# Nick-qsv/MLP-PPO-2PLY-P3

Measured on AMD Instinct MI355X. Metric: self-play env steps/sec (whole node) + 2-ply evals/sec at batch=65536, higher is better.
Workload: dtype int8 boards / fp32-equivalent policy MLP (split-f16 MFMA); 1 GPU; C3: B=65536 games/GPU PPO rollout step (policy 198->128->{500,1} + masked sample + env.step, rollout rows stored to an HBM ring); global_batch=65536, games_per_gpu=65536, max_legal_moves=500, parallelism=dp1 (independent game shards), streams_per_gpu=4, step_fork=False

## Files before the change

### mlp-ppo-2ply-p3_amd/csrc/bg_debug.h

```cpp
#pragma once
#include <string>

std::string bgx_dbg(const char* name);
long long bgx_dbg_int(const char* name, long long dflt);
```

### mlp-ppo-2ply-p3_amd/csrc/bg_engine.hip

```cpp
#include <hip/hip_runtime.h>
#include <stdio.h>
#include <stdint.h>
#include <string.h>
#include <stdlib.h>
#include <algorithm>
#include <cmath>
#include <mutex>
#include <string>
#include <vector>

#include "bg_engine.h"
#include "bg_rollout.h"
#include "bg_debug.h"
#include "bg_host.h"
#include <map>

using namespace bg;

namespace {

constexpr int kMaxRegions = BGX_MAX_COPY_REGIONS;
using namespace bg;

template <int PHASE, int LOG, int MEMO, bool NO_DOUBLES = false, int DICE = -1, bool BLK = false>
// ... 558 lines not shown
    }
    for_each_group(fin, g, [&](int gl, bool mine, uint64_t m) {
        int64_t* row = tally + (size_t)gl * 8;
        tally_add(row, BGX_ROLLOUT_GAMES, (long long)__popcll(m));
        tally_add(row, BGX_ROLLOUT_PLIES, wave_sum(mine ? p : 0));
        #pragma unroll
        for (int f = BGX_ROLLOUT_WIN1; f <= BGX_ROLLOUT_LOSS3; ++f) tally_add(row, f, count(mine && field == f));
    });
    tally_add(active, 0, -count(retired));
}

__global__ __launch_bounds__(256) void k_rollout_luck_add(const uint8_t* recs, const uint8_t* starts,
                                                          const int32_t* plies, const uint8_t* sel, const float* luck,
                                                          int n, float* lane_luck) {
    const int i = blockIdx.x * 256 + threadIdx.x;
    if (i >= n || !sel[i]) return;
    if (plies[i] == 0 && starts[(size_t)i * 64 + R_ROLL0] != 0) return;
    const float l = luck[i];
    lane_luck[i] += recs[(size_t)i * 64 + R_CUR] == starts[(size_t)i * 64 + R_CUR] ? l : -l;
}

__global__ __launch_bounds__(256) void k_rollout_luck_flush(const uint8_t* starts, const int32_t* group,
                                                            const uint8_t* sel, const uint8_t* done,
                                                            const int32_t* info, int n, int n_groups,
                                                            float* lane_luck, int64_t* luck_tally) {
    const int i = blockIdx.x * 256 + threadIdx.x;
    const bool on = i < n && sel[i] != 0;
    const int g = on ? rollout_group(group, i, n_groups) : -1;
    const bool dn = on && done[i] != 0;
    int winner, score;
    result_of(dn ? info[i] : 0, &winner, &score);
    const bool fin = dn && g >= 0 && winner >= 0;
    long long lq = 0, res = 0;
    if (fin) {
        lq = luck_q(lane_luck[i]);
        res = winner == (int)(starts[(size_t)i * 64 + R_CUR] & 1) ? score : -score;
    }
    if (dn) lane_luck[i] = 0.0f;
    for_each_group(fin, g, [&](int gl, bool mine, uint64_t m) {
        const long long v = mine ? lq : 0;
        int64_t* row = luck_tally + (size_t)gl * 4;
        tally_add(row, BGX_ROLLOUT_LUCK, wave_sum(v));
        tally_add(row, BGX_ROLLOUT_LUCK2, wave_sum(v * v));
        tally_add(row, BGX_ROLLOUT_RESLUCK, wave_sum(mine ? res * lq : 0));
        tally_add(row, BGX_ROLLOUT_LUCK_GAMES, (long long)__popcll(m));
    });
}

__device__ __forceinline__ uint64_t mix64(uint64_t x) {
    x ^= x >> 33; x *= 0xFF51AFD7ED558CCDull;
    x ^= x >> 33; x *= 0xC4CEB9FE1A85EC53ull;
    x ^= x >> 33;
    return x;
}

__global__ __launch_bounds__(256) void k_random_act(const uint8_t* recs, int n, uint64_t seed, uint32_t step,
                                                    int32_t* act) {
    const int i = blockIdx.x * 256 + threadIdx.x;
    if (i >= n) return;
    const uint32_t cnt = (uint32_t)recs[(size_t)i * 64 + R_NM0] | ((uint32_t)recs[(size_t)i * 64 + R_NM1] << 8);
    const uint64_t h = mix64(mix64(seed ^ 0x9E3779B97F4A7C15ull) + (((uint64_t)step << 32) | (uint32_t)i));
    act[i] = (int32_t)(((h >> 32) * (uint64_t)cnt) >> 32);
}

thread_local std::string g_err;

}

int bgx_internal_fail(hipError_t e, int code) {
    g_err = hipGetErrorString(e);
    return code;
}
void bgx_set_error(const char* msg) { g_err = msg; }
static std::mutex g_dbg_mu;
static std::map<std::string, std::string> g_dbg;
std::string bgx_dbg(const char* name) {
    std::lock_guard<std::mutex> g(g_dbg_mu);
    const auto it = g_dbg.find(name);
    return it == g_dbg.end() ? std::string() : it->second;
}
long long bgx_dbg_int(const char* name, long long dflt) {
    const std::string v = bgx_dbg(name);
    return v.empty() ? dflt : strtoll(v.c_str(), nullptr, 10);
}

#define LAUNCH_LOG(K, grid, s, ...) hipLaunchKernelGGL(K<9>, grid, dim3(64), 0, s, __VA_ARGS__)

static void launch_count(bgx_engine* e, hipStream_t s) {
    const int ncnt = (e->a.B + kCountThreads - 1) / kCountThreads;
    hipLaunchKernelGGL(k_order_count, dim3(ncnt), dim3(kCountThreads), 0, s, e->a.pre, e->a.cls, e->a.ctr, e->a.key0, e->a.key1,
                       e->order_cnt, e->a.B, e->ovf_base + 4 * (e->ovf_parity ^ 1), e->a.xcd);
    e->ovf_next_zeroed = true;
    e->gather_due = true;
}

static void launch_gather(bgx_engine* e, hipStream_t s, const int32_t* actions) {
    const Args& A = e->a;
    const int nblk = (A.B + kGatherThreads - 1) / kGatherThreads, ncnt = (A.B + kCountThreads - 1) / kCountThreads;
    if (actions)
        hipLaunchKernelGGL(k_step_gather<true>, dim3(nblk), dim3(kGatherThreads), 0, s, A.cls, e->order_cnt, e->perm, A.B,
                           ncnt, A.xcd, A.moves, A.ctr, actions, A.max_moves, e->blk);
    else
        hipLaunchKernelGGL(k_step_gather<false>, dim3(nblk), dim3(kGatherThreads), 0, s, A.cls, e->order_cnt, e->perm, A.B,
                           ncnt, A.xcd, nullptr, nullptr, nullptr, 0, nullptr);
}

struct StepIo {
    const int32_t* actions;
    float *obs, *reward;
    uint8_t* done;
    int32_t* info;
};

static void launch_heavy(hipStream_t s, const Args& a, int grid, const StepIo& io) {
    if (grid <= 0) return;
    if (a.blk)
        hipLaunchKernelGGL((k_step<0, 9, 0, false, 1, BGX_DICE_PHILOX, true>), dim3(grid), dim3(64), 0, s, a, io.actions,
                           io.obs, io.reward, io.done, io.info, 0);
    else if (a.dice_mode == BGX_DICE_PHILOX)
        hipLaunchKernelGGL((k_step<0, 9, 0, false, 1, BGX_DICE_PHILOX>), dim3(grid), dim3(64), 0, s, a, io.actions,
                           io.obs, io.reward, io.done, io.info, 0);
    else
        hipLaunchKernelGGL((k_step<0, 9, 0>), dim3(grid), dim3(64), 0, s, a, io.actions, io.obs, io.reward, io.done,
                           io.info, 0);
}

static void launch_light(hipStream_t s, const Args& a, int heavy, const StepIo& io) {
    hipLaunchKernelGGL((k_step<0, 8, 0, true, 1, BGX_DICE_PHILOX, true>), dim3(a.B - heavy), dim3(64), 0, s, a, io.actions,
                       io.obs, io.reward, io.done, io.info, heavy);
}

static int heavy_grid(int B, bool xcd) {
    const double g = B / 6.0 + 4.0 * std::sqrt(B * 5.0 / 36.0) + 32.0;
    int h = g >= B ? B : (int)g;
    if (xcd) h = (h + 7) & ~7;
    return h > B ? B : h;
}

static int slow_path(bgx_engine* e, hipStream_t s, int src, const int8_t* boards, const uint8_t* players,
                     const uint8_t* dice, int cap, int16_t* nm, int32_t* nt, uint64_t* moves) {
    if (src == 0)
        hipLaunchKernelGGL(k_movegen_over<0>, dim3(e->slow_waves), dim3(64), 0, s, e->a, boards, players, dice, cap,
                           nm, nt, moves, e->slow_tables);
    else
        hipLaunchKernelGGL(k_movegen_over<1>, dim3(e->slow_waves), dim3(64), 0, s, e->a, boards, players, dice, cap,
                           nm, nt, moves, e->slow_tables);
    return bgx_launch_status();
}

struct EngineBuf {
    void** p;
    size_t bytes;
    bool zero;
};
static std::vector<EngineBuf> engine_bufs(bgx_engine* e, bool stamps, bool order) {
    Args& A = e->a;
    const size_t B = (size_t)A.B;
    const bool shared = A.dice_mode == BGX_DICE_MT_SHARED;
    return {
        {(void**)&A.lanes, B * 64, true},
        {(void**)&A.moves, B * (size_t)A.max_moves * 8, false},
        {(void**)&A.n_total, B * 4, true},
        {(void**)&A.mt, (A.dice_mode == BGX_DICE_MT_LANE ? B : 1) * kMtWords * 4, false},
        {(void**)&A.ctr, B * 8, true},
        {(void**)&A.shared_rolls, B * 4, false},
        {(void**)&e->ovf_base, 32, true},
// ... 578 lines not shown
```

### mlp-ppo-2ply-p3_amd/csrc/bg_mlp.hip

```cpp
#include <hip/hip_runtime.h>
#include <stdint.h>
#include <stdlib.h>
#include "bg_host.h"
#include "bg_debug.h"


namespace {

constexpr int kW1Ahead = 2;

typedef float f32x16 __attribute__((ext_vector_type(16)));
typedef _Float16 f16x8 __attribute__((ext_vector_type(8)));

constexpr int kIn = 198;
constexpr int kKB1 = (kIn + 15) / 16;
constexpr float kMaskLog = -103.27892990343185f;
constexpr int kHdr = 16;

__device__ __forceinline__ int lane_id() { return threadIdx.x & 63; }

__host__ __device__ inline int kperm_src(int kb, int h, int i) {
    if (kb < 12) {
        const int p = kb >= 6 ? 1 : 0;
        const int pt = 4 * (kb - 6 * p) + 2 * h + (i >> 2);
// ... 12 lines not shown
            const int n = rec[base + q];
            f[4 * q + 0] = n >= 1 ? (_Float16)1.0f : (_Float16)0.0f;
            f[4 * q + 1] = n >= 2 ? (_Float16)1.0f : (_Float16)0.0f;
            f[4 * q + 2] = n >= 3 ? (_Float16)1.0f : (_Float16)0.0f;
            f[4 * q + 3] = (_Float16)(n >= 3 ? (float)(n - 3) * 0.5f : 0.0f);
        }
    } else {
        const bool on = h == 0;
        f[0] = on ? (_Float16)((float)rec[48] * 0.5f) : (_Float16)0.0f;
        f[1] = on ? (_Float16)(float)rec[50] : (_Float16)0.0f;
        f[2] = on ? (_Float16)((float)rec[49] * 0.5f) : (_Float16)0.0f;
        f[3] = on ? (_Float16)(float)rec[51] : (_Float16)0.0f;
        f[4] = on && rec[52] == 0 ? (_Float16)1.0f : (_Float16)0.0f;
        f[5] = on && rec[52] != 0 ? (_Float16)1.0f : (_Float16)0.0f;
        f[6] = (_Float16)0.0f;
        f[7] = (_Float16)0.0f;
    }
    return f;
}

__device__ __forceinline__ void split(float x, _Float16& hi, _Float16& lo) {
    hi = (_Float16)x;
    lo = (_Float16)(x - (float)hi);
}

__device__ __forceinline__ f16x8 as_h8(uint4 v) { return __builtin_bit_cast(f16x8, v); }

__device__ __forceinline__ int scale_exp(float max_abs) {
    if (!(max_abs > 0.0f) || !(max_abs < INFINITY)) return 0;
    int q;
    (void)frexpf(max_abs, &q);
    const int e = 14 - q;
    return e < -100 ? -100 : (e > 100 ? 100 : e);
}

__device__ __forceinline__ uint32_t mix32(uint32_t x) {
    x ^= x >> 16; x *= 0x7FEB352Du; x ^= x >> 15; x *= 0x846CA68Bu; x ^= x >> 16;
    return x;
}

__device__ __forceinline__ float fast_ln(float x) { return __builtin_amdgcn_logf(x) * 0.69314718055994531f; }
__device__ __forceinline__ float fast_exp(float x) { return __builtin_amdgcn_exp2f(x * 1.4426950408889634f); }

constexpr float kGumbelMax = 17.0f;

__device__ __forceinline__ float gumbel(uint32_t w) {
    const float u = ((float)(w >> 9) + 0.5f) * (1.0f / 8388608.0f);
    const float v = 1.0f - u;
    const float series = v * (1.0f + v * (0.5f + v * (1.0f / 3.0f)));
    const float e = v < (1.0f / 64.0f) ? series : -fast_ln(u);
    return -fast_ln(e);
}

__device__ __forceinline__ int hid(int r, int h) { return (r & 3) + 8 * (r >> 2) + 4 * h; }

struct PackView {
    const int* hdr;
    const uint4* w1q;
    const float* b1p;
    const uint4* w2q;
    const float* b2p;
};

__host__ __device__ inline int sz_w1q(int T) { return kKB1 * T * 2 * 64 * 4; }
__host__ __device__ inline int sz_b1p(int T) { return T * 16 * 64; }
__host__ __device__ inline int sz_w2q(int T, int OT) { return OT * T * 2 * 2 * 64 * 4; }
__host__ __device__ inline int sz_b2p(int OT) { return OT * 16 * 64; }

template <typename P>
__host__ __device__ inline void views(P base, int T, int OT, P& hdr, P& w1q, P& b1p, P& w2q, P& b2p) {
    hdr = base;
    w1q = hdr + kHdr;
    b1p = w1q + sz_w1q(T);
    w2q = b1p + sz_b1p(T);
    b2p = w2q + sz_w2q(T, OT);
}

constexpr int kZWin = 256, kZCap = 64;
constexpr int kHeavyDefault = 64;
constexpr int kRowBestDefault = 2;

#ifdef BGX_POLICY_STAMPS
constexpr int kStampWaves = 8192;
__device__ unsigned long long g_pstamp[kStampWaves][6];
#define PSTAMP(k) do { if (MODE == 0 && sw < kStampWaves && lane_id() == 0) g_pstamp[sw][k] = __builtin_amdgcn_s_memrealtime(); } while (0)
#else
#define PSTAMP(k) do { } while (0)
#endif
constexpr float kSkipMargin = 30.0f;

template <int T, int MODE>
__global__ __launch_bounds__(MODE == 0 ? 256 : 64) __attribute__((amdgpu_waves_per_eu(2))) void k_policy_act(const uint8_t* __restrict__ recs, int n,
                                                   const float* __restrict__ packed, int n_actions, int n_otiles,
                                                   uint32_t seed_lo, uint32_t seed_hi, uint32_t step_arg,
                                                   const uint32_t* __restrict__ step_ctr, int greedy_arg,
                                                   int32_t* act_out, float* logp_out, float* value_out,
                                                   float* logits_arg, uint8_t* records_out, int skip_arg) {
#ifdef BGX_POLICY_STAMPS
    const int sw = (int)(blockIdx.x * (MODE == 0 ? 4 : 1) + (threadIdx.x >> 6));
#endif
    PSTAMP(0);
    const uint32_t step = step_arg + (step_ctr ? *step_ctr : 0u);
    constexpr int kW = MODE == 0 ? 4 : 1;
    const bool greedy = MODE < 0 ? (greedy_arg & 1) != 0 : false;
    const int rowbest = (greedy_arg >> 1) & 3;
    float* const logits_out = MODE < 0 ? logits_arg : nullptr;
    const bool skip_on = MODE == 0 && skip_arg != 0;
    __shared__ uint8_t srec_[kW][32 * 64];
    __shared__ int zl[MODE == 0 ? kZCap : 1];
    const float *hdrf, *w1f, *b1p, *w2f, *b2p;
    views(packed, T, n_otiles, hdrf, w1f, b1p, w2f, b2p);
    const uint4* w1q = (const uint4*)w1f;
    const uint4* w2q = (const uint4*)w2f;
    const int e1 = __builtin_bit_cast(int, hdrf[0]), e2 = __builtin_bit_cast(int, hdrf[1]);
    const int l = lane_id();
    const int j = l & 31, h = l >> 5;
    const int wv = kW > 1 ? __builtin_amdgcn_readfirstlane((int)(threadIdx.x >> 6)) : 0;
    uint8_t* const srec = srec_[wv];
    const int n_extra = skip_on ? 2 * ((n + kZWin - 1) / kZWin) : 0;
    const bool extra = (int)blockIdx.x < n_extra;
    const int row0 = (((int)blockIdx.x - n_extra) * kW + wv) * 32;
    if (!extra && row0 >= n) return;
    int nzw = 0;
    if (skip_on) {
        const int base = (extra ? (int)blockIdx.x >> 1 : row0 / kZWin) * kZWin;
        uint16_t cw[kZWin / 64];
        #pragma unroll
        for (int k = 0; k < kZWin / 64; ++k)
            cw[k] = *(const uint16_t*)(recs + (size_t)min(base + 64 * k + l, n - 1) * 64 + 60);
        #pragma unroll
        for (int k = 0; k < kZWin / 64; ++k) {
            const int r = base + 64 * k + l;
            const bool z = r < n && (cw[k] == 0 || (int)cw[k] > skip_arg);
            const uint64_t m = __ballot(z);
            const int pos = nzw + __popcll(m & ((1ull << l) - 1ull));
            if (extra && wv == 0 && z && pos < kZCap) zl[pos] = r;
            nzw += __popcll(m);
        }
    }
    const int kx = extra ? ((int)blockIdx.x & 1) : 0;
    const int nz = extra ? min(nzw - 32 * kx, 32) : 32;
    if (extra && (nzw > kZCap || nz <= 0)) return;
    const bool self_zero = skip_on && !extra && nzw > kZCap;
    const int vt = n_actions >> 5;
    if (extra) __syncthreads();
    {
        const int r = l >> 1, off = (l & 1) * 32;
        const int gr = extra ? zl[32 * kx + (r < nz ? r : 0)] : (row0 + r < n ? row0 + r : n - 1);
        const uint4* src = (const uint4*)(recs + (size_t)gr * 64 + off);
        uint4* dst = (uint4*)(srec + r * 64 + off);
        const uint4 v0 = src[0], v1 = src[1];
        dst[0] = v0;
        dst[1] = v1;
        if (!extra && records_out && row0 + r < n) {
            uint4* o = (uint4*)(records_out + (size_t)(row0 + r) * 64 + off);
            o[0] = v0;
            o[1] = v1;
        }
    }
    if (kW > 1) __builtin_amdgcn_wave_barrier(); else __syncthreads();
    const uint8_t* myrec = srec + j * 64;
    const int count = (int)myrec[60] | ((int)myrec[61] << 8);
    const bool gathered = skip_on && !extra && !self_zero && (count == 0 || count > skip_arg);
    const bool row_ok = extra ? j < nz : row0 + j < n;
    const int grow = extra ? zl[32 * kx + (j < nz ? j : 0)] : row0 + j;
    const int per = extra ? (n_otiles + kW - 1) / kW : n_otiles;
    const int o_beg = extra ? min(wv * per, n_otiles) : 0, o_end = extra ? min(o_beg + per, n_otiles) : n_otiles;

    PSTAMP(1);
    f32x16 x1[T];
    constexpr int kPD = kW1Ahead;
    if (kW > 1 && extra) {
        f32x16 acc;
        if (wv < T) {
            #pragma unroll
            for (int r = 0; r < 16; ++r) acc[r] = b1p[(wv * 16 + r) * 64 + l];
            uint4 wr[kPD + 1][2];
            #pragma unroll
            for (int p = 0; p < kPD; ++p)
                #pragma unroll
                for (int f = 0; f < 2; ++f) wr[p][f] = w1q[(p * 2 * T + 2 * wv + f) * 64 + l];
            #pragma unroll
            for (int kb = 0; kb < kKB1; ++kb) {
                if (kb + kPD < kKB1) {
                    #pragma unroll
                    for (int f = 0; f < 2; ++f)
                        wr[(kb + kPD) % (kPD + 1)][f] = w1q[((kb + kPD) * 2 * T + 2 * wv + f) * 64 + l];
                }
                __builtin_amdgcn_sched_barrier(0);
                const f16x8 bf = feats8(myrec, kb, h);
                acc = __builtin_amdgcn_mfma_f32_32x32x16_f16(as_h8(wr[kb % (kPD + 1)][1]), bf, acc, 0, 0, 0);
                acc = __builtin_amdgcn_mfma_f32_32x32x16_f16(as_h8(wr[kb % (kPD + 1)][0]), bf, acc, 0, 0, 0);
            }
        }
        float* const xs = (float*)&srec_[0][0];
        #pragma unroll
        for (int t0 = 0; t0 < T; t0 += 2) {
            __syncthreads();
            if (wv >= t0 && wv < t0 + 2 && wv < T) {
                #pragma unroll
                for (int r = 0; r < 16; ++r) xs[((wv - t0) * 16 + r) * 64 + l] = acc[r];
            }
            __syncthreads();
            #pragma unroll
            for (int t = t0; t < t0 + 2 && t < T; ++t)
                #pragma unroll
                for (int r = 0; r < 16; ++r) x1[t][r] = xs[((t - t0) * 16 + r) * 64 + l];
        }
    } else {
        #pragma unroll
        for (int t = 0; t < T; ++t)
            #pragma unroll
            for (int r = 0; r < 16; ++r) x1[t][r] = b1p[(t * 16 + r) * 64 + l];
        uint4 wf[kPD + 1][2 * T];
        #pragma unroll
        for (int p = 0; p < kPD; ++p)
            #pragma unroll
            for (int f = 0; f < 2 * T; ++f) wf[p][f] = w1q[(p * 2 * T + f) * 64 + l];
        #pragma unroll
        for (int kb = 0; kb < kKB1; ++kb) {
            if (kb + kPD < kKB1) {
                #pragma unroll
                for (int f = 0; f < 2 * T; ++f) wf[(kb + kPD) % (kPD + 1)][f] = w1q[((kb + kPD) * 2 * T + f) * 64 + l];
            }
            __builtin_amdgcn_sched_barrier(0);
            const f16x8 bf = feats8(myrec, kb, h);
            #pragma unroll
            for (int t = 0; t < T; ++t) {
                const f16x8 ah = as_h8(wf[kb % (kPD + 1)][2 * t + 0]);
                const f16x8 al = as_h8(wf[kb % (kPD + 1)][2 * t + 1]);
                x1[t] = __builtin_amdgcn_mfma_f32_32x32x16_f16(al, bf, x1[t], 0, 0, 0);
                x1[t] = __builtin_amdgcn_mfma_f32_32x32x16_f16(ah, bf, x1[t], 0, 0, 0);
            }
        }
    }
    float mx = 0.0f, hn2 = 0.0f;
    #pragma unroll
    for (int t = 0; t < T; ++t)
        #pragma unroll
        for (int r = 0; r < 16; ++r) {
            x1[t][r] = fmaxf(x1[t][r], 0.0f);
            mx = fmaxf(mx, x1[t][r]);
            if (skip_on) hn2 = fmaf(x1[t][r], x1[t][r], hn2);
        }
    #pragma unroll
    for (int d = 1; d < 64; d <<= 1) mx = fmaxf(mx, __shfl_xor(mx, d));
    int o_s = n_otiles;
    float ub = INFINITY;
    if (skip_on && !extra) {
        int cm = gathered ? 0 : count;
        #pragma unroll
        for (int d = 1; d < 32; d <<= 1) cm = max(cm, __shfl_xor(cm, d));
        o_s = max((cm + 31) >> 5, 1);
        hn2 += __shfl_xor(hn2, 32);
        const float u0 = hdrf[2] + hdrf[3] * ldexpf(sqrtf(hn2), -e1);
        ub = u0 + 1e-3f * fabsf(u0) + 1e-3f;
    }
    const int ex = scale_exp(mx);
    f16x8 xh[T][2], xl[T][2];
    #pragma unroll
    for (int t = 0; t < T; ++t)
        #pragma unroll
        for (int m = 0; m < 2; ++m)
            #pragma unroll
            for (int i = 0; i < 8; ++i) {
                _Float16 a, b;
                split(ldexpf(x1[t][8 * m + i], ex), a, b);
                xh[t][m][i] = a; xl[t][m][i] = b;
            }
    const int E = e2 + e1 + ex;
    const float up = ldexpf(1.0f, E), down = ldexpf(1.0f, -E);

    PSTAMP(2);
    float m = -INFINITY, s = 0.0f, best = -INFINITY, bestz = 0.0f, value = 0.0f;
    int besta = 0;
#ifdef BGX_POLICY_STAMPS
    unsigned long long ptiles = 0;
#endif
    const uint32_t rowkey = mix32(mix32(seed_lo ^ mix32(seed_hi + 0x9E3779B9u)) ^ step) ^ (uint32_t)grow * 0x85EBCA6Bu;
    constexpr int NF = T * 2 * 2;
    uint4 w[NF];
    float bq[16];
    if (o_beg < o_end) {
        #pragma unroll
        for (int f = 0; f < NF; ++f) w[f] = w2q[((size_t)o_beg * NF + f) * 64 + l];
        #pragma unroll
        for (int r = 0; r < 16; ++r) bq[r] = b2p[(o_beg * 16 + r) * 64 + l];
    } else {
        #pragma unroll
        for (int f = 0; f < NF; ++f) w[f] = make_uint4(0, 0, 0, 0);
        #pragma unroll
        for (int r = 0; r < 16; ++r) bq[r] = 0.0f;
    }
    for (int o = o_beg; o < o_end;) {
        f32x16 y;
        #pragma unroll
        for (int r = 0; r < 16; ++r) y[r] = bq[r] * up;
        #pragma unroll
        for (int t = 0; t < T; ++t)
            #pragma unroll
            for (int mm = 0; mm < 2; ++mm) {
                const f16x8 ah = as_h8(w[(t * 2 + mm) * 2 + 0]);
                const f16x8 al = as_h8(w[(t * 2 + mm) * 2 + 1]);
                y = __builtin_amdgcn_mfma_f32_32x32x16_f16(al, xh[t][mm], y, 0, 0, 0);
                y = __builtin_amdgcn_mfma_f32_32x32x16_f16(ah, xl[t][mm], y, 0, 0, 0);
                y = __builtin_amdgcn_mfma_f32_32x32x16_f16(ah, xh[t][mm], y, 0, 0, 0);
            }
        const bool at_s = o + 1 == o_s && o_s < vt;
        const int nx = at_s ? vt : o + 1;
        __asm__ volatile("" ::: "memory");
        if (nx < o_end) {
            #pragma unroll
            for (int f = 0; f < NF; ++f) w[f] = w2q[((size_t)nx * NF + f) * 64 + l];
        }
        float z[16];
        float tm = -INFINITY;
        #pragma unroll
        for (int r = 0; r < 16; ++r) {
            const int a = 32 * o + hid(r, h);
            const float z0 = y[r] * down;
            if (logits_out && row_ok && a <= n_actions) logits_out[(size_t)grow * (32 * n_otiles) + a] = z0;
            value = a == n_actions ? z0 : value;
            z[r] = a < n_actions ? (a < count ? z0 : z0 + kMaskLog) : -INFINITY;
            tm = fmaxf(tm, z[r]);
        }
        __asm__ volatile("" ::: "memory");
        if (nx < o_end) {
            #pragma unroll
            for (int r = 0; r < 16; ++r) bq[r] = b2p[(nx * 16 + r) * 64 + l];
        }
        const float mn = fmaxf(m, tm);
        if (mn != -INFINITY) {
            float acc = 0.0f;
            #pragma unroll
            for (int r = 0; r < 16; ++r) acc += fast_exp(z[r] - mn);
            s = s * fast_exp(m - mn) + acc;
            m = mn;
        }
        const float b_row = rowbest ? fmaxf(best, __shfl_xor(best, 32)) : best;
#ifdef BGX_POLICY_STAMPS
        bool drawn = false;
#endif
        #pragma unroll
        for (int g = 0; g < 4; ++g) {
            const float gm = !greedy && rowbest == 2
                ? fmaxf(fmaxf(z[4 * g], z[4 * g + 1]), fmaxf(z[4 * g + 2], z[4 * g + 3])) : tm;
            const bool draw = greedy ? gm > best : !(gm + kGumbelMax < fmaxf(b_row, best)) && !(rowbest && gathered);
#ifdef BGX_POLICY_STAMPS
            drawn = drawn || draw;
#endif
            if (draw) {
                #pragma unroll
                for (int r = 4 * g; r < 4 * g + 4; ++r) {
                    const int a = 32 * o + hid(r, h);
                    const float key = greedy ? z[r] : z[r] + gumbel(mix32(rowkey ^ ((uint32_t)a * 0xC2B2AE35u)));
                    const bool up_ = key > best;
                    best = up_ ? key : best;
                    besta = up_ ? a : besta;
                    bestz = up_ ? z[r] : bestz;
                }
            }
        }
#ifdef BGX_POLICY_STAMPS
        if (MODE == 0) {
            const unsigned long long any = __ballot(drawn) != 0ull;
            ptiles += 1ull + (any << 8);
            ptiles |= any && o == vt ? 1ull << 16 : 0ull;
            ptiles |= any && o >= o_s && o != vt ? 1ull << 17 : 0ull;
        }
#endif
        int next = o + 1;
        if (at_s) {
            const float m_row = fmaxf(m, __shfl_xor(m, 32)), b_row = fmaxf(best, __shfl_xor(best, 32));
            const bool ok = gathered || (ub + kMaskLog < m_row - kSkipMargin && ub + kMaskLog + kGumbelMax < b_row);
            if (__ballot(!ok) == 0ull) {
                next = vt;
            } else {
                int o1 = o + 1;
                __asm__ volatile("" : "+v"(o1));
                #pragma unroll
                for (int f = 0; f < NF; ++f) w[f] = w2q[((size_t)o1 * NF + f) * 64 + l];
                #pragma unroll
                for (int r = 0; r < 16; ++r) bq[r] = b2p[(o1 * 16 + r) * 64 + l];
            }
        }
        o = next;
    }
    if (kW > 1 && extra) {
        __shared__ float pm[kW > 1 ? kW - 1 : 1][5][64];
        __shared__ int pa[kW > 1 ? kW - 1 : 1][64];
        if (wv > 0) {
            pm[wv - 1][0][l] = m; pm[wv - 1][1][l] = s; pm[wv - 1][2][l] = best; pm[wv - 1][3][l] = bestz;
            pm[wv - 1][4][l] = value; pa[wv - 1][l] = besta;
        }
        __syncthreads();
        if (wv > 0) return;
        #pragma unroll
        for (int q = 0; q < kW - 1; ++q) {
            const float mq = pm[q][0][l], sq = pm[q][1][l], bq = pm[q][2][l], zq = pm[q][3][l];
            const int aq = pa[q][l];
            const float mn = fmaxf(m, mq);
            if (mn != -INFINITY) s = s * fast_exp(m - mn) + sq * fast_exp(mq - mn);
            m = mn;
            const bool tk = bq > best || (bq == best && aq < besta);
            best = tk ? bq : best;
            besta = tk ? aq : besta;
            bestz = tk ? zq : bestz;
            value += pm[q][4][l];
        }
    }
    PSTAMP(3);
#ifdef BGX_POLICY_STAMPS
    if (MODE == 0 && sw < kStampWaves && lane_id() == 0) {
        g_pstamp[sw][4] = extra ? 1 : 2;
        g_pstamp[sw][5] = ptiles;
    }
#endif
    const float m2 = __shfl_xor(m, 32), s2 = __shfl_xor(s, 32);
    const float best2 = __shfl_xor(best, 32), bestz2 = __shfl_xor(bestz, 32);
    const int besta2 = __shfl_xor(besta, 32);
    const float value2 = __shfl_xor(value, 32);
    const float mm = fmaxf(m, m2);
    const float ss = s * fast_exp(m - mm) + s2 * fast_exp(m2 - mm);
    const bool take2 = best2 > best || (best2 == best && besta2 < besta);
    const int a_fin = take2 ? besta2 : besta;
    const float z_fin = take2 ? bestz2 : bestz;
    const float v_fin = h == 0 ? value + value2 : 0.0f;
    if (h == 0 && row_ok && !gathered) {
        act_out[grow] = a_fin;
        if (logp_out) logp_out[grow] = fminf(fmaxf(z_fin - (mm + logf(ss)), -15.942384719848633f),
                                             -1.1920930376163597e-07f);
        if (value_out) value_out[grow] = v_fin;
    }
}

__global__ __launch_bounds__(1024) void k_policy_scale(const float* W1, const float* Wa, const float* ba,
                                                       const float* wv, int H, int A, float* hdr) {
    __shared__ float r1[16], r2[16], r3[16], r4[16];
    const int t = threadIdx.x;
    float m1 = 0.0f, m2 = 0.0f, bmax = -INFINITY, nmax = 0.0f;
    for (int i = t; i < H * kIn; i += 1024) m1 = fmaxf(m1, fabsf(W1[i]));
    for (int i = t; i < A * H; i += 1024) m2 = fmaxf(m2, fabsf(Wa[i]));
    for (int i = t; i < H; i += 1024) m2 = fmaxf(m2, fabsf(wv[i]));
    for (int a = t; a < A; a += 1024) {
        double q = 0.0;
        for (int k = 0; k < H; ++k) q += (double)Wa[(size_t)a * H + k] * (double)Wa[(size_t)a * H + k];
        nmax = fmaxf(nmax, (float)sqrt(q));
        bmax = fmaxf(bmax, ba[a]);
    }
    #pragma unroll
    for (int d = 1; d < 64; d <<= 1) {
        m1 = fmaxf(m1, __shfl_xor(m1, d)); m2 = fmaxf(m2, __shfl_xor(m2, d));
        bmax = fmaxf(bmax, __shfl_xor(bmax, d)); nmax = fmaxf(nmax, __shfl_xor(nmax, d));
    }
    if ((t & 63) == 0) { r1[t >> 6] = m1; r2[t >> 6] = m2; r3[t >> 6] = bmax; r4[t >> 6] = nmax; }
    __syncthreads();
    if (t == 0) {
        for (int w = 1; w < 16; ++w) {
            m1 = fmaxf(m1, r1[w]); m2 = fmaxf(m2, r2[w]); bmax = fmaxf(bmax, r3[w]); nmax = fmaxf(nmax, r4[w]);
        }
        hdr[0] = __builtin_bit_cast(float, scale_exp(m1));
        hdr[1] = __builtin_bit_cast(float, scale_exp(m2));
        hdr[2] = bmax;
        hdr[3] = nmax * (1.0f + 1.0f / 1024.0f);
        for (int i = 4; i < kHdr; ++i) hdr[i] = 0.0f;
    }
}

__global__ void k_policy_pack(const float* W1, const float* b1, const float* Wa, const float* ba, const float* wv,
                              const float* bv, int H, int A, int T, int OT, float* packed) {
    float *hdr, *w1f, *b1p, *w2f, *b2p;
    views(packed, T, OT, hdr, w1f, b1p, w2f, b2p);
    const int e1 = __builtin_bit_cast(int, hdr[0]), e2 = __builtin_bit_cast(int, hdr[1]);
    _Float16* w1h = (_Float16*)w1f;
    _Float16* w2h = (_Float16*)w2f;
    const int tid = blockIdx.x * blockDim.x + threadIdx.x;
    const int n1 = kKB1 * T * 64 * 8, nb1 = T * 16 * 64, n2 = OT * T * 2 * 64 * 8, nb2 = OT * 16 * 64;
    auto W2 = [&](int o, int k) -> float {
        if (k >= H) return 0.0f;
        if (o < A) return Wa[(size_t)o * H + k];
        if (o == A) return wv[k];
        return 0.0f;
    };
    auto B2 = [&](int o) -> float { return o < A ? ba[o] : (o == A ? bv[0] : 0.0f); };
    if (tid < n1) {
        const int i = tid % 8, l = (tid / 8) % 64, t = (tid / 512) % T, kb = tid / (512 * T);
        const int hrow = 32 * t + (l & 31), k = kperm_src(kb, l >> 5, i);
        const float wk = hrow < H && k >= 0 ? W1[(size_t)hrow * kIn + k] : 0.0f;
        const float w = ldexpf(k == 97 || k == 195 ? wk / 15.0f : wk, e1);
        _Float16 a, b;
        split(w, a, b);
        w1h[(((kb * T + t) * 2 + 0) * 64 + l) * 8 + i] = a;
        w1h[(((kb * T + t) * 2 + 1) * 64 + l) * 8 + i] = b;
    } else if (tid < n1 + nb1) {
        const int q = tid - n1;
        const int l = q % 64, r = (q / 64) % 16, t = q / (64 * 16);
        const int hrow = 32 * t + hid(r, l >> 5);
        b1p[q] = hrow < H ? ldexpf(b1[hrow], e1) : 0.0f;
// ... 159 lines not shown
    const int H = a.hidden, A = a.n_actions;
    if (a.bound) {
        const int r = blockIdx.x * 4 + (threadIdx.x >> 6), l = threadIdx.x & 63;
        if (r < A) {
            float s = 0.0f;
            for (int c = l; c < H; c += 64) {
                const float v = (float)(_Float16)a.wa[(size_t)r * H + c];
                s = fmaf(v, v, s);
            }
            #pragma unroll
            for (int o = 32; o >= 1; o >>= 1) s += __shfl_xor(s, o);
            if (l == 0) {
                a.bound[r] = sqrtf(s);
                a.bound[512 + r] = fabsf((float)(_Float16)a.ba[r]);
            }
        }
    }
    const long long n0 = (long long)kKB1 * a.T * 64, n1 = n0 + H, n2 = n1 + 512LL * H, n3 = n2 + 512,
                    n4 = n3 + (long long)H * 208, n5 = n4 + 512LL * H, n6 = n5 + 512, n7 = n6 + 1;
    for (long long g = (long long)blockIdx.x * 256 + threadIdx.x; g < n7; g += (long long)gridDim.x * 256) {
        if (g < n0) {
            const int l = (int)(g & 63), t = (int)((g >> 6) % a.T), kb = (int)((g >> 6) / a.T);
            const int u = 32 * t + (l & 31);
            f16x8 v;
            #pragma unroll
            for (int i = 0; i < 8; ++i) {
                const int src = kperm_src(kb, l >> 5, i);
                v[i] = (u < H && src >= 0) ? (_Float16)a.w1[(size_t)u * kIn + src] : (_Float16)0.0f;
            }
            a.w1pack[g] = __builtin_bit_cast(uint4, v);
        } else if (g < n1) {
            const int u = (int)(g - n0);
            a.b1h[u] = (_Float16)a.b1[u];
        } else if (g < n2) {
            const long long e = g - n1;
            const int r = (int)(e / H), c = (int)(e % H);
            a.w2h[e] = r < A ? (_Float16)a.wa[(size_t)r * H + c] : (r == A ? (_Float16)a.wv[c] : (_Float16)0.0f);
        } else if (g < n3) {
            const int r = (int)(g - n2);
            a.b2h[r] = r < A ? (_Float16)a.ba[r] : (r == A ? (_Float16)a.bv[0] : (_Float16)0.0f);
        } else if (g < n4) {
            a.gw1[g - n3] = 0.0f;
        } else if (g < n5) {
            a.gw2[g - n4] = 0.0f;
        } else if (g < n6) {
            a.gb2[g - n5] = 0.0f;
        } else if (a.hmax2) {
            a.hmax2[0] = 0.0f;
        }
    }
    if (a.sums && blockIdx.x == 0 && threadIdx.x < 3) a.sums[threadIdx.x] = 0.0;
}

__global__ void k_counter_add(uint32_t* ctr, uint32_t v) {
    if (threadIdx.x == 0) *ctr += v;
}

}

extern "C" {

int bgx_policy_packed_size(int32_t hidden, int32_t n_actions) {
    if (hidden <= 0 || hidden > 128 || n_actions <= 0) return BGX_EINVAL;
    const int T = (hidden + 31) / 32, OT = (n_actions + 1 + 31) / 32;
    return kHdr + sz_w1q(T) + sz_b1p(T) + sz_w2q(T, OT) + sz_b2p(OT);
}

int bgx_policy_pack(const float* W1, const float* b1, const float* Wa, const float* ba, const float* wv, const float* bv,
                    int32_t hidden, int32_t n_actions, float* packed, void* stream) {
    const int total = bgx_policy_packed_size(hidden, n_actions);
    if (total < 0 || !W1 || !b1 || !Wa || !ba || !wv || !bv || !packed) return BGX_EINVAL;
    const int T = (hidden + 31) / 32, OT = (n_actions + 1 + 31) / 32;
    hipStream_t s = (hipStream_t)stream;
    hipLaunchKernelGGL(k_policy_scale, dim3(1), dim3(1024), 0, s, W1, Wa, ba, wv, hidden, n_actions, packed);
    const int work = kKB1 * T * 64 * 8 + T * 16 * 64 + OT * T * 2 * 64 * 8 + OT * 16 * 64;
    hipLaunchKernelGGL(k_policy_pack, dim3((work + 255) / 256), dim3(256), 0, s, W1, b1, Wa, ba, wv, bv, hidden,
                       n_actions, T, OT, packed);
    return bgx_launch_status();
}

#ifdef BGX_POLICY_STAMPS
extern "C" int bgx_debug_policy_stamps(unsigned long long* out, int32_t waves) {
    if (hipDeviceSynchronize() != hipSuccess) return BGX_EDEVICE;
    if (hipMemcpyFromSymbol(out, HIP_SYMBOL(g_pstamp), (size_t)(waves < kStampWaves ? waves : kStampWaves) * 48) != hipSuccess)
        return BGX_EDEVICE;
    static unsigned long long z[kStampWaves][6];
    return hipMemcpyToSymbol(HIP_SYMBOL(g_pstamp), z, sizeof z) == hipSuccess ? BGX_OK : BGX_EDEVICE;
}
#endif

int bgx_policy_act_ctr(const uint8_t* records_dev, int32_t n, const float* packed, int32_t hidden, int32_t n_actions,
                       uint64_t seed, uint32_t step, const uint32_t* step_ctr, int32_t greedy, int32_t* act_out,
                       float* logp_out, float* value_out, float* logits_out, uint8_t* records_out, void* stream) {
    if (bgx_policy_packed_size(hidden, n_actions) < 0 || n < 0 || (n > 0 && (!records_dev || !packed || !act_out)))
        return BGX_EINVAL;
    if (n == 0) return BGX_OK;
    const int T = (hidden + 31) / 32, OT = (n_actions + 1 + 31) / 32;
    const int n_main = (n + 31) / 32;
    const dim3 grid(n_main), blk(64);
    const int n_wg = (n + 127) / 128;
    hipStream_t s = (hipStream_t)stream;
    const uint32_t lo = (uint32_t)seed, hi = (uint32_t)(seed >> 32);
    const bool plain = !greedy && !logits_out;
    const bool skip = bgx_dbg_int("BGX_POLICY_SKIP", 1) != 0;
    const int heavy = (int)bgx_dbg_int("BGX_POLICY_HEAVY", kHeavyDefault);
    const int garg = (greedy ? 1 : 0) | ((int)min(max(bgx_dbg_int("BGX_POLICY_ROWBEST", kRowBestDefault), 0ll), 2ll) << 1);
    const dim3 grid0(skip ? n_wg + 2 * ((n + kZWin - 1) / kZWin) : n_wg);
#define BGX_ACT(TT)                                                                                           \
    do {                                                                                                      \
        if (plain)                                                                                            \
            hipLaunchKernelGGL((k_policy_act<TT, 0>), grid0, dim3(256), 0, s, records_dev, n, packed, n_actions, OT, \
                               lo, hi, step, step_ctr, garg, act_out, logp_out, value_out, logits_out,     \
                               records_out, skip ? (heavy > 0 ? heavy : 1) : 0);                             \
        else                                                                                                  \
            hipLaunchKernelGGL((k_policy_act<TT, -1>), grid, blk, 0, s, records_dev, n, packed, n_actions, OT,   \
                               lo, hi, step, step_ctr, garg, act_out, logp_out, value_out, logits_out,     \
                               records_out, 0);                                                               \
    } while (0)
    switch (T) {
        case 1: BGX_ACT(1); break;
        case 2: BGX_ACT(2); break;
        case 3: BGX_ACT(3); break;
        default: BGX_ACT(4); break;
    }
#undef BGX_ACT
    return bgx_launch_status();
}

int bgx_policy_act_rec(const uint8_t* records_dev, int32_t n, const float* packed, int32_t hidden, int32_t n_actions,
                       uint64_t seed, uint32_t step, int32_t greedy, int32_t* act_out, float* logp_out,
                       float* value_out, float* logits_out, uint8_t* records_out, void* stream) {
    return bgx_policy_act_ctr(records_dev, n, packed, hidden, n_actions, seed, step, nullptr, greedy, act_out, logp_out,
                              value_out, logits_out, records_out, stream);
}

int bgx_counter_add(uint32_t* ctr_dev, uint32_t v, void* stream) {
    if (!ctr_dev) return BGX_EINVAL;
    hipLaunchKernelGGL(k_counter_add, dim3(1), dim3(64), 0, (hipStream_t)stream, ctr_dev, v);
    return bgx_launch_status();
}

int bgx_policy_act(const uint8_t* records_dev, int32_t n, const float* packed, int32_t hidden, int32_t n_actions,
                   uint64_t seed, uint32_t step, int32_t greedy, int32_t* act_out, float* logp_out, float* value_out,
                   float* logits_out, void* stream) {
    return bgx_policy_act_rec(records_dev, n, packed, hidden, n_actions, seed, step, greedy, act_out, logp_out,
                              value_out, logits_out, nullptr, stream);
}

int bgx_fc1_packed_size(int32_t hidden) {
    if (hidden <= 0 || hidden > 128 || hidden % 4) return BGX_EINVAL;
    return kKB1 * ((hidden + 31) / 32) * 64 * 16;
}

int bgx_fc1_pack(const void* w1h_dev, int32_t hidden, void* packed_dev, void* stream) {
    if (bgx_fc1_packed_size(hidden) < 0 || !w1h_dev || !packed_dev) return BGX_EINVAL;
    if ((uintptr_t)packed_dev % 16) return BGX_EINVAL;
    const int T = (hidden + 31) / 32, work = kKB1 * T * 64;
    hipLaunchKernelGGL(k_fc1_pack, dim3((work + 255) / 256), dim3(256), 0, (hipStream_t)stream,
                       (const _Float16*)w1h_dev, hidden, T, (uint4*)packed_dev);
    return bgx_launch_status();
}

int bgx_ppo_epoch_prep(const float* w1_dev, const float* b1_dev, const float* wa_dev, const float* ba_dev,
                       const float* wv_dev, const float* bv_dev, int32_t hidden, int32_t n_actions, void* w1pack_dev,
                       void* b1h_dev, void* w2h_dev, void* b2h_dev, float* gw1_dev, float* gw2_dev, float* gb2_dev,
                       float* hmax2_dev_or_null, float* bound_dev_or_null, double* sums_dev_or_null, void* stream) {
    if (bgx_fc1_packed_size(hidden) < 0 || n_actions <= 0 || n_actions >= 512) return BGX_EINVAL;
    if (!w1_dev || !b1_dev || !wa_dev || !ba_dev || !wv_dev || !bv_dev || !w1pack_dev || !b1h_dev || !w2h_dev ||
        !b2h_dev || !gw1_dev || !gw2_dev || !gb2_dev || (uintptr_t)w1pack_dev % 16)
        return BGX_EINVAL;
    EpochPrep a{w1_dev, b1_dev, wa_dev, ba_dev, wv_dev, bv_dev, hidden, n_actions, (hidden + 31) / 32,
                (uint4*)w1pack_dev, (_Float16*)b1h_dev, (_Float16*)w2h_dev, (_Float16*)b2h_dev, gw1_dev, gw2_dev,
                gb2_dev, hmax2_dev_or_null, bound_dev_or_null, sums_dev_or_null};
    hipLaunchKernelGGL(k_ppo_epoch_prep, dim3(512), dim3(256), 0, (hipStream_t)stream, a);
    return bgx_launch_status();
}

int bgx_fc1_records(const uint8_t* records_dev, int32_t n, const void* packed_dev, const void* b1h_dev,
                    int32_t hidden, void* h_dev, void* stream) {
    return bgx_fc1_records_ex(records_dev, n, packed_dev, b1h_dev, hidden, h_dev, nullptr, stream);
}

int bgx_fc1_records_ex(const uint8_t* records_dev, int32_t n, const void* packed_dev, const void* b1h_dev,
                       int32_t hidden, void* h_dev, float* hmax2_dev, void* stream) {
    if (bgx_fc1_packed_size(hidden) < 0 || n < 0 || (n > 0 && (!records_dev || !packed_dev || !b1h_dev || !h_dev)))
        return BGX_EINVAL;
    if (((uintptr_t)records_dev | (uintptr_t)packed_dev) % 16 || (uintptr_t)h_dev % 8) return BGX_EINVAL;
    if (n == 0) return BGX_OK;
    const int T = (hidden + 31) / 32;
// ... 17 lines not shown
```

Baseline: 552.2 million env steps/s.

## Compact live rows per wave, add value-only final tile, batch debug option lookups

In the policy-act kernel, each wave now builds a compacted list of live (non-skipped) rows within its 256-row window, sorted by legal-move count. Waves therefore process dense groups of rows with similar move counts instead of fixed contiguous slices, and waves with no live rows exit early. Once every action tile has been pruned, a value-only path loads just the value-head weight column and extracts the value without computing the full last tile. Host-side option parsing is collapsed into one locked map lookup that returns immediately when no debug options are set. The row indirection and extra ballots add instruction and register cost, and records are now written in scattered rather than contiguous order.

Result: no change. 553.6 million env steps/s (median of 2 runs) (+0.3%).

```diff
diff --git a/mlp-ppo-2ply-p3_amd/csrc/bg_debug.h b/mlp-ppo-2ply-p3_amd/csrc/bg_debug.h
--- a/mlp-ppo-2ply-p3_amd/csrc/bg_debug.h
+++ b/mlp-ppo-2ply-p3_amd/csrc/bg_debug.h
@@ -3,3 +3,4 @@
 
 std::string bgx_dbg(const char* name);
 long long bgx_dbg_int(const char* name, long long dflt);
+void bgx_dbg_ints(const char* const* names, long long* vals, int n);
diff --git a/mlp-ppo-2ply-p3_amd/csrc/bg_engine.hip b/mlp-ppo-2ply-p3_amd/csrc/bg_engine.hip
--- a/mlp-ppo-2ply-p3_amd/csrc/bg_engine.hip
+++ b/mlp-ppo-2ply-p3_amd/csrc/bg_engine.hip
@@ -664,6 +664,14 @@
 long long bgx_dbg_int(const char* name, long long dflt) {
     const std::string v = bgx_dbg(name);
     return v.empty() ? dflt : strtoll(v.c_str(), nullptr, 10);
+}
+void bgx_dbg_ints(const char* const* names, long long* vals, int n) {
+    std::lock_guard<std::mutex> g(g_dbg_mu);
+    if (g_dbg.empty()) return;
+    for (int i = 0; i < n; ++i) {
+        const auto it = g_dbg.find(names[i]);
+        if (it != g_dbg.end() && !it->second.empty()) vals[i] = strtoll(it->second.c_str(), nullptr, 10);
+    }
 }
 
 #define LAUNCH_LOG(K, grid, s, ...) hipLaunchKernelGGL(K<9>, grid, dim3(64), 0, s, __VA_ARGS__)
diff --git a/mlp-ppo-2ply-p3_amd/csrc/bg_mlp.hip b/mlp-ppo-2ply-p3_amd/csrc/bg_mlp.hip
--- a/mlp-ppo-2ply-p3_amd/csrc/bg_mlp.hip
+++ b/mlp-ppo-2ply-p3_amd/csrc/bg_mlp.hip
@@ -118,7 +118,7 @@
 
 #ifdef BGX_POLICY_STAMPS
 constexpr int kStampWaves = 8192;
-__device__ unsigned long long g_pstamp[kStampWaves][6];
+__device__ unsigned long long g_pstamp[kStampWaves][8];
 #define PSTAMP(k) do { if (MODE == 0 && sw < kStampWaves && lane_id() == 0) g_pstamp[sw][k] = __builtin_amdgcn_s_memrealtime(); } while (0)
 #else
 #define PSTAMP(k) do { } while (0)
@@ -157,13 +157,17 @@
     const bool extra = (int)blockIdx.x < n_extra;
     const int row0 = (((int)blockIdx.x - n_extra) * kW + wv) * 32;
     if (!extra && row0 >= n) return;
-    int nzw = 0;
+    __shared__ int pl[MODE == 0 ? kW : 1][32];
+    const bool part_on = skip_on && (greedy_arg & 16) != 0;
+    int nzw = 0, nlv = 0;
     if (skip_on) {
         const int base = (extra ? (int)blockIdx.x >> 1 : row0 / kZWin) * kZWin;
         uint16_t cw[kZWin / 64];
         #pragma unroll
         for (int k = 0; k < kZWin / 64; ++k)
             cw[k] = *(const uint16_t*)(recs + (size_t)min(base + 64 * k + l, n - 1) * 64 + 60);
+        uint64_t ma[kZWin / 64] = {}, mb[kZWin / 64] = {};
+        int na = 0;
         #pragma unroll
         for (int k = 0; k < kZWin / 64; ++k) {
             const int r = base + 64 * k + l;
@@ -172,24 +176,49 @@
             const int pos = nzw + __popcll(m & ((1ull << l) - 1ull));
             if (extra && wv == 0 && z && pos < kZCap) zl[pos] = r;
             nzw += __popcll(m);
+            if (part_on && !extra) {
+                const bool live = r < n && !z;
+                ma[k] = __ballot(live && cw[k] <= 32);
+                mb[k] = __ballot(live && cw[k] > 32);
+                na += __popcll(ma[k]);
+            }
+        }
+        if (part_on && !extra && nzw <= kZCap) {
+            const int p0 = ((row0 % kZWin) >> 5) * 32;
+            const uint64_t below = (1ull << l) - 1ull;
+            int ca = 0, cb = na;
+            #pragma unroll
+            for (int k = 0; k < kZWin / 64; ++k) {
+                const bool a = (ma[k] >> l) & 1ull, b = (mb[k] >> l) & 1ull;
+                const int pos = (a ? ca + __popcll(ma[k] & below) : cb + __popcll(mb[k] & below)) - p0;
+                if ((a || b) && pos >= 0 && pos < 32) pl[wv][pos] = base + 64 * k + l;
+                ca += __popcll(ma[k]);
+                cb += __popcll(mb[k]);
+            }
+            nlv = cb - p0;
         }
     }
     const int kx = extra ? ((int)blockIdx.x & 1) : 0;
-    const int nz = extra ? min(nzw - 32 * kx, 32) : 32;
+    const bool self_zero = skip_on && !extra && nzw > kZCap;
+    const bool part = part_on && !extra && !self_zero;
+    const int nz = extra ? min(nzw - 32 * kx, 32) : part ? min(nlv, 32) : 32;
     if (extra && (nzw > kZCap || nz <= 0)) return;
-    const bool self_zero = skip_on && !extra && nzw > kZCap;
+    if (part && nz <= 0) return;
     const int vt = n_actions >> 5;
     if (extra) __syncthreads();
+    if (part) __builtin_amdgcn_wave_barrier();
+    const bool listed = extra || part;
+    const int* const lst = extra ? zl + 32 * kx : pl[wv];
     {
         const int r = l >> 1, off = (l & 1) * 32;
-        const int gr = extra ? zl[32 * kx + (r < nz ? r : 0)] : (row0 + r < n ? row0 + r : n - 1);
+        const int gr = listed ? lst[r < nz ? r : 0] : (row0 + r < n ? row0 + r : n - 1);
         const uint4* src = (const uint4*)(recs + (size_t)gr * 64 + off);
         uint4* dst = (uint4*)(srec + r * 64 + off);
         const uint4 v0 = src[0], v1 = src[1];
         dst[0] = v0;
         dst[1] = v1;
-        if (!extra && records_out && row0 + r < n) {
-            uint4* o = (uint4*)(records_out + (size_t)(row0 + r) * 64 + off);
+        if (records_out && (extra ? part_on && wv == 0 && r < nz : part ? r < nz : row0 + r < n)) {
+            uint4* o = (uint4*)(records_out + (size_t)gr * 64 + off);
             o[0] = v0;
             o[1] = v1;
         }
@@ -198,8 +227,8 @@
     const uint8_t* myrec = srec + j * 64;
     const int count = (int)myrec[60] | ((int)myrec[61] << 8);
     const bool gathered = skip_on && !extra && !self_zero && (count == 0 || count > skip_arg);
-    const bool row_ok = extra ? j < nz : row0 + j < n;
-    const int grow = extra ? zl[32 * kx + (j < nz ? j : 0)] : row0 + j;
+    const bool row_ok = listed ? j < nz : row0 + j < n;
+    const int grow = listed ? lst[j < nz ? j : 0] : row0 + j;
     const int per = extra ? (n_otiles + kW - 1) / kW : n_otiles;
     const int o_beg = extra ? min(wv * per, n_otiles) : 0, o_end = extra ? min(o_beg + per, n_otiles) : n_otiles;
 
@@ -328,6 +357,12 @@
         #pragma unroll
         for (int r = 0; r < 16; ++r) bq[r] = 0.0f;
     }
+    const bool valpass = MODE == 0 && skip_on && !extra && !self_zero && (greedy_arg & 8) != 0;
+    const int vr = n_actions & 31, r_v = (vr & 3) + 4 * (vr >> 3), h_v = (vr >> 2) & 1;
+    bool vonly = false;
+#ifdef BGX_POLICY_STAMPS
+    unsigned long long t_tile = __builtin_amdgcn_s_memrealtime(), t_act = 0, t_val = 0;
+#endif
     for (int o = o_beg; o < o_end;) {
         f32x16 y;
         #pragma unroll
@@ -342,10 +377,29 @@
                 y = __builtin_amdgcn_mfma_f32_32x32x16_f16(ah, xl[t][mm], y, 0, 0, 0);
                 y = __builtin_amdgcn_mfma_f32_32x32x16_f16(ah, xh[t][mm], y, 0, 0, 0);
             }
+        if (MODE == 0 && vonly) {
+            int rv = r_v;
+            __asm__ volatile("" : "+s"(rv));
+            float v = 0.0f;
+            #pragma unroll
+            for (int r = 0; r < 16; ++r) v = r == rv ? y[r] : v;
+            value = h == h_v ? v * down : value;
+#ifdef BGX_POLICY_STAMPS
+            t_val += __builtin_amdgcn_s_memrealtime() - t_tile;
+            ptiles |= 1ull << 18;
+#endif
+            break;
+        }
         const bool at_s = o + 1 == o_s && o_s < vt;
         const int nx = at_s ? vt : o + 1;
+        const bool at_v = MODE == 0 && at_s && valpass;
         __asm__ volatile("" ::: "memory");
-        if (nx < o_end) {
+        if (at_v) {
+            if (j == vr) {
+                #pragma unroll
+                for (int f = 0; f < NF; ++f) w[f] = w2q[((size_t)nx * NF + f) * 64 + l];
+            }
+        } else if (nx < o_end) {
             #pragma unroll
             for (int f = 0; f < NF; ++f) w[f] = w2q[((size_t)nx * NF + f) * 64 + l];
         }
@@ -361,7 +415,11 @@
             tm = fmaxf(tm, z[r]);
         }
         __asm__ volatile("" ::: "memory");
-        if (nx < o_end) {
+        if (at_v) {
+            const float bv = b2p[(nx * 16 + r_v) * 64 + l];
+            #pragma unroll
+            for (int r = 0; r < 16; ++r) bq[r] = bv;
+        } else if (nx < o_end) {
             #pragma unroll
             for (int r = 0; r < 16; ++r) bq[r] = b2p[(nx * 16 + r) * 64 + l];
         }
@@ -411,6 +469,7 @@
             const bool ok = gathered || (ub + kMaskLog < m_row - kSkipMargin && ub + kMaskLog + kGumbelMax < b_row);
             if (__ballot(!ok) == 0ull) {
                 next = vt;
+                vonly = at_v;
             } else {
                 int o1 = o + 1;
                 __asm__ volatile("" : "+v"(o1));
@@ -420,6 +479,13 @@
                 for (int r = 0; r < 16; ++r) bq[r] = b2p[(o1 * 16 + r) * 64 + l];
             }
         }
+#ifdef BGX_POLICY_STAMPS
+        {
+            const unsigned long long t_now = __builtin_amdgcn_s_memrealtime();
+            (o == vt ? t_val : t_act) += t_now - t_tile;
+            t_tile = t_now;
+        }
+#endif
         o = next;
     }
     if (kW > 1 && extra) {
@@ -450,6 +516,8 @@
     if (MODE == 0 && sw < kStampWaves && lane_id() == 0) {
         g_pstamp[sw][4] = extra ? 1 : 2;
         g_pstamp[sw][5] = ptiles;
+        g_pstamp[sw][6] = t_act;
+        g_pstamp[sw][7] = t_val;
     }
 #endif
     const float m2 = __shfl_xor(m, 32), s2 = __shfl_xor(s, 32);
@@ -775,9 +843,9 @@
 #ifdef BGX_POLICY_STAMPS
 extern "C" int bgx_debug_policy_stamps(unsigned long long* out, int32_t waves) {
     if (hipDeviceSynchronize() != hipSuccess) return BGX_EDEVICE;
-    if (hipMemcpyFromSymbol(out, HIP_SYMBOL(g_pstamp), (size_t)(waves < kStampWaves ? waves : kStampWaves) * 48) != hipSuccess)
+    if (hipMemcpyFromSymbol(out, HIP_SYMBOL(g_pstamp), (size_t)(waves < kStampWaves ? waves : kStampWaves) * sizeof g_pstamp[0]) != hipSuccess)
         return BGX_EDEVICE;
-    static unsigned long long z[kStampWaves][6];
+    static unsigned long long z[kStampWaves][8];
     return hipMemcpyToSymbol(HIP_SYMBOL(g_pstamp), z, sizeof z) == hipSuccess ? BGX_OK : BGX_EDEVICE;
 }
 #endif
@@ -795,9 +863,14 @@
     hipStream_t s = (hipStream_t)stream;
     const uint32_t lo = (uint32_t)seed, hi = (uint32_t)(seed >> 32);
     const bool plain = !greedy && !logits_out;
-    const bool skip = bgx_dbg_int("BGX_POLICY_SKIP", 1) != 0;
-    const int heavy = (int)bgx_dbg_int("BGX_POLICY_HEAVY", kHeavyDefault);
-    const int garg = (greedy ? 1 : 0) | ((int)min(max(bgx_dbg_int("BGX_POLICY_ROWBEST", kRowBestDefault), 0ll), 2ll) << 1);
+    static const char* const kOpts[5] = {"BGX_POLICY_SKIP", "BGX_POLICY_HEAVY", "BGX_POLICY_ROWBEST", "BGX_POLICY_VALUE",
+                                         "BGX_POLICY_PART"};
+    long long opt[5] = {1, kHeavyDefault, kRowBestDefault, 1, 1};
+    bgx_dbg_ints(kOpts, opt, 5);
+    const bool skip = opt[0] != 0;
+    const int heavy = (int)opt[1];
+    const int garg = (greedy ? 1 : 0) | ((int)min(max(opt[2], 0ll), 2ll) << 1) | (opt[3] != 0 ? 8 : 0) |
+                     (opt[4] != 0 ? 16 : 0);
     const dim3 grid0(skip ? n_wg + 2 * ((n + kZWin - 1) / kZWin) : n_wg);
 #define BGX_ACT(TT)                                                                                           \
     do {                                                                                                      \
```
